# nv-tlabs/ASE

Hardware: AMD Instinct MI355X
Metric: ASE PPO-update samples/sec (4096 envs x horizon 32) (higher is better)
Workload: dtype f16; 1 GPU; BASELINE configs[1]: ASE agent, 4096 envs x horizon 32, obs 253 / act 31 / amp obs 1400 / latent 64, [1024,1024,512] MLPs + disc + shared-trunk encoder, minibatch 16384 (amp 4096) x 6 mini-epochs = 48 optimisation steps per update; random-init weights; precision_choice=auto without an oracle leg: the first candidate, replay=program, parallelism=single GPU

## Files before the change

ase_amd/csrc/gemm_nt_kernels.h:

```cpp
#pragma once
#include "gemm_nt.h"
#include <stdlib.h>
#include <utility>

namespace {

using namespace ase_nt;

typedef uint32_t u32x4 __attribute__((ext_vector_type(4)));
template <int N, typename F, int... I> __device__ __forceinline__ void static_for_impl(F&& f, std::integer_sequence<int, I...>) {
    (f(std::integral_constant<int, I>{}), ...);
}
template <int N, typename F> __device__ __forceinline__ void static_for(F&& f) { static_for_impl<N>(f, std::make_integer_sequence<int, N>{}); }

template <typename T> struct Mma;

template <typename T> struct Mma16 {
    typedef typename V16<T>::x8 x8;
    template <int FM, int FN, int RB, bool SW = false>
    static __device__ __forceinline__ void tile(const char* sA, const char* sB, int lane, f32x16 (&acc)[FM][FN]) {
        const int r = lane & 31, h = lane >> 5, sw = lds_swz<RB>(r);
#pragma unroll
        for (int ks = 0; ks < RB / 32; ++ks) {
            x8 a[FM], b[FN];
            const int off = r * RB + (((ks * 2 + h) ^ sw) << 4);
#pragma unroll
            for (int i = 0; i < FM; ++i)
                a[i] = *reinterpret_cast<const x8*>(sA + i * 32 * RB + off);
#pragma unroll
            for (int j = 0; j < FN; ++j)
                b[j] = *reinterpret_cast<const x8*>(sB + j * 32 * RB + off);
#pragma unroll
            for (int i = 0; i < FM; ++i)
#pragma unroll
                for (int j = 0; j < FN; ++j) {
                    if constexpr (SW) acc[i][j] = mfma16<T>(b[j], a[i], acc[i][j]);
                    else acc[i][j] = mfma16<T>(a[i], b[j], acc[i][j]);
                }
        }
    }
};
template <> struct Mma<bf16_t> : Mma16<bf16_t> {};
template <> struct Mma<f16_t> : Mma16<f16_t> {};

template <> struct Mma<float> {
    template <int FM, int FN, int RB>
    static __device__ __forceinline__ void tile(const char* sA, const char* sB, int lane, f32x16 (&acc)[FM][FN]) {
        const int r = lane & 31, h = lane >> 5, sw = lds_swz<RB>(r);
#pragma unroll
        for (int kb = 0; kb < RB / 32; ++kb) {
            f32x4 a[FM], b[FN];
            const int off = r * RB + (((kb * 2 + h) ^ sw) << 4);
#pragma unroll
            for (int i = 0; i < FM; ++i)
                a[i] = *reinterpret_cast<const f32x4*>(sA + i * 32 * RB + off);
#pragma unroll
            for (int j = 0; j < FN; ++j)
                b[j] = *reinterpret_cast<const f32x4*>(sB + j * 32 * RB + off);
#pragma unroll
            for (int e = 0; e < 4; ++e)
#pragma unroll
                for (int i = 0; i < FM; ++i)
#pragma unroll
                    for (int j = 0; j < FN; ++j)
                        acc[i][j] = __builtin_amdgcn_mfma_f32_32x32x2f32(a[i][e], b[j][e], acc[i][j], 0, 0, 0);
        }
    }
};

__device__ __forceinline__ void split_bf16(const f32x4& x0, const f32x4& x1, bf16x8& hi, bf16x8& lo) {
#pragma unroll
    for (int q = 0; q < 4; ++q) {
        hi[q] = (bf16_t)x0[q];
        hi[q + 4] = (bf16_t)x1[q];
        lo[q] = (bf16_t)(x0[q] - (float)hi[q]);
        lo[q + 4] = (bf16_t)(x1[q] - (float)hi[q + 4]);
    }
}

template <> struct Mma<f32s_t> {
    template <int FM, int FN, int RB>
    static __device__ __forceinline__ void tile(const char* sA, const char* sB, int lane, f32x16 (&acc)[FM][FN]) {
        const int r = lane & 31, h = lane >> 5, sw = lds_swz<RB>(r);
#pragma unroll
        for (int ks = 0; ks < RB / 64; ++ks) {
            bf16x8 ah[FM], al[FM], bh[FN], bl[FN];
            const int c0 = ks * 4 + h * 2;
            const int o0 = r * RB + ((c0 ^ sw) << 4), o1 = r * RB + (((c0 + 1) ^ sw) << 4);
#pragma unroll
            for (int i = 0; i < FM; ++i)
                split_bf16(*reinterpret_cast<const f32x4*>(sA + i * 32 * RB + o0),
                           *reinterpret_cast<const f32x4*>(sA + i * 32 * RB + o1), ah[i], al[i]);
#pragma unroll
            for (int j = 0; j < FN; ++j)
                split_bf16(*reinterpret_cast<const f32x4*>(sB + j * 32 * RB + o0),
                           *reinterpret_cast<const f32x4*>(sB + j * 32 * RB + o1), bh[j], bl[j]);
#pragma unroll
            for (int i = 0; i < FM; ++i)
#pragma unroll
                for (int j = 0; j < FN; ++j) {
                    acc[i][j] = __builtin_amdgcn_mfma_f32_32x32x16_bf16(al[i], bh[j], acc[i][j], 0, 0, 0);
                    acc[i][j] = __builtin_amdgcn_mfma_f32_32x32x16_bf16(ah[i], bl[j], acc[i][j], 0, 0, 0);
                    acc[i][j] = __builtin_amdgcn_mfma_f32_32x32x16_bf16(ah[i], bh[j], acc[i][j], 0, 0, 0);
                }
        }
    }
};

__device__ __forceinline__ void split_f16_pair(float x0, float x1, float sa, uint32_t& hi, uint32_t& lo) {
    asm("v_fma_mixlo_f16 %0, %4, %2, 0\n\t"
        "v_fma_mixhi_f16 %0, %4, %3, 0\n\t"
        "v_fma_mixlo_f16 %1, %4, %2, -%0 op_sel_hi:[0,0,1]\n\t"
        "v_fma_mixhi_f16 %1, %4, %3, -%0 op_sel:[0,0,1] op_sel_hi:[0,0,1]"
        : "=&v"(hi), "=&v"(lo)
        : "v"(x0), "v"(x1), "s"(sa));
}
__device__ __forceinline__ void split_f16_fence(u32x4& hi, u32x4& lo) { asm("s_nop 1" : "+v"(hi), "+v"(lo)); }

template <> struct Mma<f32h_t> {
    template <int RB>
    static __device__ __forceinline__ void frag_offsets(int lane, uint32_t a0, uint32_t b0, uint32_t (&fa)[RB / 64][2], uint32_t (&fb)[RB / 64][2]) {
        const int r = lane & 31, h = lane >> 5, sw = lds_swz<RB>(r);
#pragma unroll
        for (int ks = 0; ks < RB / 64; ++ks)
#pragma unroll
            for (int c = 0; c < 2; ++c) {
                const uint32_t o = r * RB + (((ks * 4 + h * 2 + c) ^ sw) << 4);
                fa[ks][c] = a0 + o;
                fb[ks][c] = b0 + o;
                asm volatile("" : "+v"(fa[ks][c]), "+v"(fb[ks][c]));
            }
    }
    template <int FM, int FN, int RB>
    static __device__ __forceinline__ void tile(const char* smem, uint32_t sbuf, const uint32_t (&fa)[RB / 64][2], const uint32_t (&fb)[RB / 64][2],
                                                f32x16 (&acc)[FM][FN], float sa) {
        constexpr int KS = RB / 64, NM = FM * FN * 3, NP = FM * 4;
        constexpr bool PF = FM * FN <= 4;
        f32x4 ax[2][FM][2];
        u32x4 ah[2][FM], al[2][FM];
        f16x8 bh[2][FN], bl[2][FN];
        auto read_a = [&](int ks) {
#pragma unroll
            for (int i = 0; i < FM; ++i)
#pragma unroll
                for (int c = 0; c < 2; ++c) ax[ks & 1][i][c] = *reinterpret_cast<const f32x4*>(smem + (fa[ks][c] + sbuf) + i * 32 * RB);
        };
        auto read_b = [&](int ks) {
#pragma unroll
            for (int j = 0; j < FN; ++j) {
                bh[PF ? ks & 1 : 0][j] = *reinterpret_cast<const f16x8*>(smem + (fb[ks][0] + sbuf) + j * 32 * RB);
                bl[PF ? ks & 1 : 0][j] = *reinterpret_cast<const f16x8*>(smem + (fb[ks][1] + sbuf) + j * 32 * RB);
            }
        };
        auto split_pair = [&](int ks, int q) {
            const int i = q >> 2, c = (q >> 1) & 1, e = (q & 1) * 2;
            uint32_t hi, lo;
            split_f16_pair(ax[ks & 1][i][c][e], ax[ks & 1][i][c][e + 1], sa, hi, lo);
            ah[ks & 1][i][c * 2 + (q & 1)] = hi;
            al[ks & 1][i][c * 2 + (q & 1)] = lo;
        };
        auto fence = [&](int ks) {
#pragma unroll
            for (int i = 0; i < FM; ++i) split_f16_fence(ah[ks & 1][i], al[ks & 1][i]);
        };
        read_a(0);
        read_b(0);
        __builtin_amdgcn_sched_barrier(0);
#pragma unroll
        for (int q = 0; q < NP; ++q) split_pair(0, q);
        fence(0);
#pragma unroll
        for (int ks = 0; ks < KS; ++ks) {
            const bool more = ks + 1 < KS;
            if (more) {
                read_a(ks + 1);
                if constexpr (PF) read_b(ks + 1);
            }
            __builtin_amdgcn_sched_barrier(0);
#pragma unroll
            for (int i = 0; i < FM; ++i)
#pragma unroll
                for (int j = 0; j < FN; ++j)
#pragma unroll
                    for (int t = 0; t < 3; ++t) {
                        const f16x8 a = __builtin_bit_cast(f16x8, t == 0 ? al[ks & 1][i] : ah[ks & 1][i]);
                        const f16x8 b = (t == 1) ? bl[PF ? ks & 1 : 0][j] : bh[PF ? ks & 1 : 0][j];
                        acc[i][j] = __builtin_amdgcn_mfma_f32_32x32x16_f16(a, b, acc[i][j], 0, 0, 0);
                        if (more) {
                            const int m = (i * FN + j) * 3 + t;
                            __builtin_amdgcn_sched_barrier(0);
#pragma unroll
                            for (int q = 0; q < NP; ++q)
                                if (q * NM >= m * NP && q * NM < (m + 1) * NP) split_pair(ks + 1, q);
                            __builtin_amdgcn_sched_barrier(0);
                        }
                    }
            if (more) {
                fence(ks + 1);
                if constexpr (!PF) read_b(ks + 1);
            }
        }
    }
};

template <int PASSES, int RPP, int RB>
__device__ __forceinline__ void nt_stage(const char* const (&src)[PASSES], int64_t koff, char* lds_wave_base) {
#pragma unroll
    for (int i = 0; i < PASSES; ++i)
        __builtin_amdgcn_global_load_lds((gptr_t*)(src[i] + koff), (lptr_t*)(lds_wave_base + i * RPP * RB), 16, 0, 0);
}
template <typename T, int AUXK> struct AuxReg;
template <typename T> struct AuxReg<T, 0> { char v; };
template <> struct AuxReg<bf16_t, 1> { bf16x4 v; };
template <> struct AuxReg<f16_t, 1> { f16x4 v; };
template <> struct AuxReg<float, 1> { f32x4 v; };
template <> struct AuxReg<f32s_t, 1> { f32x4 v; };
template <> struct AuxReg<f32h_t, 1> { f32x4 v; };
template <typename T> struct AuxReg<T, 2> { uint32_t v; };

__device__ __forceinline__ uint32_t or8_dpp(uint32_t x) {
    x |= (uint32_t)__builtin_amdgcn_update_dpp(0, (int)x, 0xB1, 0xF, 0xF, true);
    x |= (uint32_t)__builtin_amdgcn_update_dpp(0, (int)x, 0x4E, 0xF, 0xF, true);
    x |= (uint32_t)__builtin_amdgcn_update_dpp(0, (int)x, 0x141, 0xF, 0xF, true);
    return x;
}

template <typename T, int FM, int FN, int FMC, int FNC, int AUXK>
__device__ __forceinline__ void nt_aux_load(const NTParams& p, int ch, int lane, int mrow0, int ncol0,
                                            AuxReg<T, AUXK> (&dst)[(FMC * 32) / (64 / (FNC * 8))]) {
    constexpr int ELPR = FNC * 8, RPI = 64 / ELPR, NIT = (FMC * 32) / RPI;
    if constexpr (AUXK != 0) {
        const int c4 = lane % ELPR, rsub = lane / ELPR;
        const int jc = (ch / (FM / FMC)) * FNC, ic = (ch % (FM / FMC)) * FMC;
        const int n0 = ncol0 + jc * 32 + c4 * 4;
#pragma unroll
        for (int it = 0; it < NIT; ++it) {
            const int m = mrow0 + ic * 32 + it * RPI + rsub;
            if (n0 < p.N && m < p.M) {
                const int ma = (m >= p.aux_split) ? m - p.aux_delta : m;
                if constexpr (AUXK == 2)
                    dst[it].v = *reinterpret_cast<const uint32_t*>(p.aux + (int64_t)ma * p.ldaux + (n0 >> 5) * 4);
                else
                    dst[it].v = *reinterpret_cast<const decltype(dst[it].v)*>(p.aux + (int64_t)ma * p.ldaux + (int64_t)n0 * sizeof(T));
            }
        }
    }
}

template <typename T, int FM, int FN, int FMC, int FNC, int AUXK, bool PRE = false, bool FUSE = false>
__device__ __forceinline__ double nt_epilogue_impl(const NTParams& p, f32x16 (&acc)[FM][FN], float* slab, int lane,
                                                   int mrow0, int ncol0,
                                                   AuxReg<T, AUXK> (*pre)[(FMC * 32) / (64 / (FNC * 8))] = nullptr) {
    constexpr int WCOLS = FNC * 32, WROWS = FMC * 32;
    const int col_in = lane & 31, row_hi = (lane >> 5) * 4;
    constexpr int ELPR = WCOLS / 4;
    constexpr int RPI = 64 / ELPR;
    constexpr int NIT = WROWS / RPI;
    constexpr int NCH = (FN / FNC) * (FM / FMC);
    constexpr bool AHEAD = AUXK != 0 && sizeof(AuxReg<T, AUXK>) <= 8;
    const int c4 = lane % ELPR, rsub = lane / ELPR;
    AuxReg<T, AUXK> areg[AHEAD ? 2 : 1][NIT];
    bool bad = false;
    double sq = 0.0;

    auto load_aux = [&](int ch, AuxReg<T, AUXK> (&dst)[NIT]) {
        nt_aux_load<T, FM, FN, FMC, FNC, AUXK>(p, ch, lane, mrow0, ncol0, dst);
    };

    if constexpr (PRE) {
#pragma unroll
        for (int it = 0; it < NIT; ++it) areg[0][it] = (*pre)[it];
    } else if constexpr (AUXK != 0) {
        load_aux(0, areg[0]);
    }
#pragma unroll
    for (int ch = 0; ch < NCH; ++ch) {
        const int jc = (ch / (FM / FMC)) * FNC, ic = (ch % (FM / FMC)) * FMC;
        const int n0 = ncol0 + jc * 32 + c4 * 4;
        if constexpr (AHEAD) {
            if (ch + 1 < NCH) load_aux(ch + 1, areg[(ch + 1) & 1]);
        } else if constexpr (AUXK != 0) {
            if (ch > 0) load_aux(ch, areg[0]);
        }
        AuxReg<T, AUXK> (&cur)[NIT] = areg[AHEAD ? (ch & 1) : 0];
#pragma unroll
        for (int jj = 0; jj < FNC; ++jj) {
            const int j = jc + jj;
            const int n = ncol0 + j * 32 + col_in;
            const float bias = (p.bias && n < p.N) ? p.bias[n] : 0.f;
#pragma unroll
            for (int ii = 0; ii < FMC; ++ii) {
#pragma unroll
                for (int e = 0; e < 16; ++e) {
                    float v = p.alpha * acc[ic + ii][j][e] + bias;
                    if (p.act == ASE_ACT_RELU) v = v <= 0.f ? 0.f : v;
                    else if (p.act == ASE_ACT_TANH) v = tanhf(v);
                    slab[(ii * 32 + row_hi + (e & 3) + 8 * (e >> 2)) * WCOLS + jj * 32 + col_in] = v;
                }
            }
        }
        float cs[4] = {0.f, 0.f, 0.f, 0.f};
        f32x4 seed = {0.f, 0.f, 0.f, 0.f};
        if constexpr (FUSE) {
            if (p.seed_w && n0 < p.N) {
#pragma unroll
                for (int q = 0; q < 4; ++q) seed[q] = p.seed_scale * (n0 + q < p.seed_n ? p.seed_w[n0 + q] : 0.f);
            }
        }
        if (n0 < p.N) {
#pragma unroll
            for (int it = 0; it < NIT; ++it) {
                const int row = it * RPI + rsub;
                const int m = mrow0 + ic * 32 + row;
                if (m >= p.M) continue;
                f32x4 v = *reinterpret_cast<const f32x4*>(slab + row * WCOLS + c4 * 4);
                if (p.act >= ASE_ACT_SILU) {
                    if (p.pre_out) {
                        if constexpr (sizeof(T) == 2) {
                            typename V16<T>::x4 zt;
#pragma unroll
                            for (int q = 0; q < 4; ++q) {
                                zt[q] = from_f32<T>(v[q]);
                                bad |= ovf_hit1(zt[q]);
                            }
                            *reinterpret_cast<typename V16<T>::x4*>(p.pre_out + (int64_t)m * p.ldpre + (int64_t)n0 * 2) = zt;
                        } else {
#pragma unroll
                            for (int q = 0; q < 4; ++q) bad |= ovf_hit1(v[q]);
                            *reinterpret_cast<f32x4*>(p.pre_out + (int64_t)m * p.ldpre + (int64_t)n0 * 4) = v;
                        }
                    }
#pragma unroll
                    for (int q = 0; q < 4; ++q) v[q] = act_apply(p.act, v[q]);
                }
                if constexpr (AUXK == 2) {
                    const uint32_t nib = cur[it].v >> (n0 & 31);
#pragma unroll
                    for (int q = 0; q < 4; ++q) v[q] = ((nib >> q) & 1u) ? v[q] : 0.f;
                } else if constexpr (AUXK == 1) {
#pragma unroll
                    for (int q = 0; q < 4; ++q) {
                        const float a = (float)cur[it].v[q];
                        if (p.aux_mode == ASE_AUX_RELU_MASK) v[q] = a > 0.f ? v[q] : 0.f;
                        else if (p.aux_mode == ASE_AUX_TANH_GRAD) v[q] = v[q] * (1.f - a * a);
                        else v[q] = v[q] * act_grad(p.aux_mode >> 8, a);
                    }
                }
                if constexpr (FUSE) {
                    f32x4 sv = v;
                    if (p.seed_w) {
#pragma unroll
                        for (int q = 0; q < 4; ++q) sv[q] = seed[q] * (v[q] > 0.f ? 1.f : 0.f);
                    }
#pragma unroll
                    for (int q = 0; q < 4; ++q) bad |= ovf_hit1(sv[q]);
                    if (p.C) *reinterpret_cast<f32x4*>(p.C + (int64_t)m * p.ldc + (int64_t)n0 * 4) = sv;
                    if (p.twin) {
                        char* t = p.twin + (int64_t)m * p.ldtwin + (int64_t)n0 * 2;
                        if (p.twin_dtype == ASE_F16) {
                            f16x4 o;
#pragma unroll
                            for (int q = 0; q < 4; ++q) o[q] = from_f32<f16_t>(sv[q]);
                            *reinterpret_cast<f16x4*>(t) = o;
                        } else {
                            bf16x4 o;
#pragma unroll
                            for (int q = 0; q < 4; ++q) o[q] = from_f32<bf16_t>(sv[q]);
                            *reinterpret_cast<bf16x4*>(t) = o;
                        }
                    }
                    if (p.sq_acc) {
                        float s = 0.f;
#pragma unroll
                        for (int q = 0; q < 4; ++q) s = __fadd_rn(s, __fmul_rn(sv[q], sv[q]));
                        sq += (double)s;
                    }
                } else if (p.out_f32 || sizeof(T) == 4) {
#pragma unroll
                    for (int q = 0; q < 4; ++q) bad |= ovf_hit1(v[q]);
                    *reinterpret_cast<f32x4*>(p.C + (int64_t)m * p.ldc + (int64_t)n0 * 4) = v;
                } else {
                    typedef typename std::conditional<sizeof(T) == 2, T, bf16_t>::type S;
                    typename V16<S>::x4 o;
#pragma unroll
                    for (int q = 0; q < 4; ++q) {
                        o[q] = from_f32<S>(v[q]);
                        bad |= ovf_hit1(o[q]);
                        v[q] = (float)o[q];
                    }
                    *reinterpret_cast<typename V16<S>::x4*>(p.C + (int64_t)m * p.ldc + (int64_t)n0 * 2) = o;
                }
#pragma unroll
                for (int q = 0; q < 4; ++q) cs[q] += v[q];
                if (p.mask_out) {
                    uint32_t bits = 0;
#pragma unroll
                    for (int q = 0; q < 4; ++q) bits |= (v[q] > 0.f ? 1u : 0u) << q;
                    bits = or8_dpp(bits << (n0 & 31));
                    if ((c4 & 7) == 0) p.mask_out[(int64_t)m * p.ldmask + (n0 >> 5)] = bits;
                }
            }
        }
        if (p.colsum) {
#pragma unroll
            for (int q = 0; q < 4; ++q) {
#pragma unroll
                for (int o = ELPR; o < 64; o <<= 1) cs[q] += __shfl_xor(cs[q], o, 64);
            }
            if (lane < ELPR) {
#pragma unroll
                for (int q = 0; q < 4; ++q)
                    if (n0 + q < p.colsum_n) atomic_add_f32(p.colsum + n0 + q, cs[q]);
            }
        }
    }
    ovf_report(p.alpha_dev, bad);
    return sq;
}

template <typename T, int FM, int FN, int FMC, int FNC, bool FUSE = false>
__device__ __forceinline__ double nt_epilogue(const NTParams& p, f32x16 (&acc)[FM][FN], float* slab, int lane, int mrow0,
                                              int ncol0) {
    if (p.aux_mode == ASE_AUX_NONE) return nt_epilogue_impl<T, FM, FN, FMC, FNC, 0, false, FUSE>(p, acc, slab, lane, mrow0, ncol0);
    if (p.aux_mode == ASE_AUX_RELU_BITS) return nt_epilogue_impl<T, FM, FN, FMC, FNC, 2, false, FUSE>(p, acc, slab, lane, mrow0, ncol0);
    if constexpr (FUSE) return 0.0;
    else return nt_epilogue_impl<T, FM, FN, FMC, FNC, 1>(p, acc, slab, lane, mrow0, ncol0);
}

template <typename T, int FM, int FN, int AUXK, bool MASK>
__device__ __forceinline__ void nt_epilogue_rows_impl(const NTParams& p, f32x16 (&acc)[FM][FN], int lane, int mrow0, int ncol0,
                                                      const uint32_t (&bits)[FM][FN]) {
    const int r = lane & 31, h = lane >> 5;
    const f32x2 al = {p.alpha, p.alpha};
    const float relu_lo = (p.act == ASE_ACT_RELU) ? 0.f : -__builtin_inff();
    uint32_t ovf = 0;
#pragma unroll
    for (int j = 0; j < FN; ++j) {
        f32x4 bias[4];
#pragma unroll
        for (int g = 0; g < 4; ++g) {
            if (p.bias) bias[g] = *reinterpret_cast<const f32x4*>(p.bias + ncol0 + j * 32 + 8 * g + 4 * h);
            else bias[g] = f32x4{0.f, 0.f, 0.f, 0.f};
        }
#pragma unroll
        for (int i = 0; i < FM; ++i) {
            const int m = mrow0 + i * 32 + r;
            const bool row_ok = m < p.M;
            char* crow = p.C + (int64_t)m * p.ldc + (int64_t)(ncol0 + j * 32) * 2 + h * 16;
            uint32_t pk[4][2];
            const uint32_t mb = rows_frag<T, AUXK, MASK>(acc[i][j], bias, AUXK == 2 ? bits[i][j] >> (4 * h) : 0u, al, relu_lo, h, pk);
#pragma unroll
            for (int g = 0; g < 4; g += 2) {
                const auto s0 = __builtin_amdgcn_permlane32_swap(pk[g][0], pk[g + 1][0], false, false);
                const auto s1 = __builtin_amdgcn_permlane32_swap(pk[g][1], pk[g + 1][1], false, false);
                if (row_ok) *reinterpret_cast<uint4*>(crow + 8 * g * 2) = make_uint4(s0[0], s1[0], s0[1], s1[1]);
                ovf = ovf_fold(ovf_fold(ovf_fold(ovf_fold(ovf, s0[0]), s1[0]), s0[1]), s1[1]);
            }
            if constexpr (MASK) {
                const auto w = __builtin_amdgcn_permlane32_swap(mb, mb, false, false);
                if (row_ok && h == 0) p.mask_out[(int64_t)m * p.ldmask + ((ncol0 + j * 32) >> 5)] = w[0] | w[1];
            }
        }
    }
    ovf_report(p.alpha_dev, ovf_hit<T>(ovf));
}

template <typename T, int FM, int FN, int AUXK>
__device__ __forceinline__ void nt_epilogue_rows(const NTParams& p, f32x16 (&acc)[FM][FN], int lane, int mrow0, int ncol0,
                                                 const uint32_t (&bits)[FM][FN]) {
    if (ncol0 >= p.N) return;
    if (p.mask_out) nt_epilogue_rows_impl<T, FM, FN, AUXK, true>(p, acc, lane, mrow0, ncol0, bits);
    else nt_epilogue_rows_impl<T, FM, FN, AUXK, false>(p, acc, lane, mrow0, ncol0, bits);
}

template <int WGM, int WGN, int FM, int FN, int RB, int S, int A_PASSES, int B_PASSES>
__device__ __forceinline__ void nt_h3_loop(const NTParams& p, char* smem, const char* const (&srcA)[A_PASSES], const char* const (&srcB)[B_PASSES],
                                           int lane, int wid, int wm, int wn, int nk, f32x16 (&acc)[FM][FN]) {
    constexpr int BM = WGM * FM * 32, BN = WGN * FN * 32, RPW = 64 / (RB / 16), RPP = WGM * WGN * RPW, P = A_PASSES + B_PASSES;
    constexpr int kBuf = (BM + BN) * RB;
    uint32_t fa[RB / 64][2], fb[RB / 64][2];
    Mma<f32h_t>::template frag_offsets<RB>(lane, (wm * FM * 32) * RB, (BM + wn * FN * 32) * RB, fa, fb);
    const bool fits32 = (int64_t)p.M * p.lda < (int64_t)0x7FFFFFFF && (int64_t)p.N * p.ldb < (int64_t)0x7FFFFFFF;
    const i32x4 rsA = raw_buffer(p.A), rsB = raw_buffer(p.B);
    const uint32_t lds0 = __builtin_amdgcn_readfirstlane((uint32_t)(uintptr_t)smem + wid * RPW * RB);
    uint32_t voffA[A_PASSES], voffB[B_PASSES];
#pragma unroll
    for (int i = 0; i < A_PASSES; ++i) voffA[i] = (uint32_t)(srcA[i] - p.A);
#pragma unroll
    for (int i = 0; i < B_PASSES; ++i) voffB[i] = (uint32_t)(srcB[i] - p.B);
    auto stage = [&](int t, int b) {
        const uint32_t dst = lds0 + (uint32_t)b * kBuf;
        if (fits32) {
            const uint32_t soff = (uint32_t)t * RB;
            static_for<A_PASSES>([&](auto i) { lds_dma16<i.value * RPP * RB, true>(dst, voffA[i.value], rsA, soff); });
            static_for<B_PASSES>([&](auto i) { lds_dma16<(BM + i.value * RPP) * RB, true>(dst, voffB[i.value], rsB, soff); });
        } else {
            const int64_t koff = (int64_t)t * RB;
            static_for<A_PASSES>([&](auto i) { lds_dma16_global<i.value * RPP * RB>(dst, srcA[i.value] + koff); });
            static_for<B_PASSES>([&](auto i) { lds_dma16_global<(BM + i.value * RPP) * RB>(dst, srcB[i.value] + koff); });
        }
    };
#pragma unroll
    for (int t = 0; t < S - 1; ++t)
        if (t < nk) stage(t, t);
    __builtin_amdgcn_s_waitcnt(0xC07F);
    int buf = 0, prev = S - 1;
    for (int kt = 0; kt < nk; ++kt) {
        if (kt + S - 2 < nk) wait_vmcnt<P*(S - 2)>();
        else wait_vmcnt<0>();
        __builtin_amdgcn_s_barrier();
        if (kt + S - 1 < nk) stage(kt + S - 1, prev);
        Mma<f32h_t>::template tile<FM, FN, RB>(smem, (uint32_t)buf * kBuf, fa, fb, acc, p.sa);
        prev = buf;
        buf = (buf + 1 == S) ? 0 : buf + 1;
    }
}

template <typename T, int WGM, int WGN, int FM, int FN, int RB, int S, int WPE = 1, bool SW = false, bool FUSE = false>
__global__ __launch_bounds__(WGM * WGN * 64, WPE) void gemm_nt_kernel(NTParams p) {
    constexpr int BM = WGM * FM * 32, BN = WGN * FN * 32;
    constexpr int BK = RB / (int)sizeof(T);
    constexpr int LPR = RB / 16;
    constexpr int RPW = 64 / LPR;
    constexpr int RPP = WGM * WGN * RPW;
    constexpr int A_PASSES = BM / RPP, B_PASSES = BN / RPP;
    constexpr int P = A_PASSES + B_PASSES;
    static_assert(BM % RPP == 0 && BN % RPP == 0, "tile rows must be a multiple of the rows staged per pass");
    extern __shared__ __attribute__((aligned(16))) char smem[];
    constexpr int kBuf = (BM + BN) * RB;
    if (p.alpha_dev) p.alpha *= *p.alpha_dev;

    const int tid = threadIdx.x, lane = tid & 63, wid = tid >> 6;
    const int wm = wid / WGN, wn = wid % WGN;
    const int nwg = p.tiles_m * p.tiles_n;
    const int tile = xcd_remap(blockIdx.x, nwg);
    const int bm0 = (tile / p.tiles_n) * BM, bn0 = (tile % p.tiles_n) * BN;

    const int srow = tid / LPR, sslot = tid % LPR;
    const char* srcA[A_PASSES];
    const char* srcB[B_PASSES];
#pragma unroll
    for (int i = 0; i < A_PASSES; ++i) {
        const int r = i * RPP + srow;
        srcA[i] = p.A + (int64_t)min(bm0 + r, p.M - 1) * p.lda + ((sslot ^ lds_swz<RB>(r)) << 4);
    }
#pragma unroll
    for (int i = 0; i < B_PASSES; ++i) {
        const int r = i * RPP + srow;
        srcB[i] = p.B + (int64_t)min(bn0 + r, p.N - 1) * p.ldb + ((sslot ^ lds_swz<RB>(r)) << 4);
    }
    char* const ldsA = smem + (wid * RPW) * RB;
    char* const ldsB = ldsA + BM * RB;

    f32x16 acc[FM][FN];
#pragma unroll
    for (int i = 0; i < FM; ++i)
#pragma unroll
        for (int j = 0; j < FN; ++j)
#pragma unroll
            for (int e = 0; e < 16; ++e) acc[i][j][e] = 0.f;

    uint32_t row_bits[FM][FN];
    auto load_bits = [&]() {
        if (p.aux_mode == ASE_AUX_RELU_BITS && bn0 + wn * FN * 32 < p.N) {
#pragma unroll
            for (int i = 0; i < FM; ++i) {
                const int m = min(bm0 + wm * FM * 32 + i * 32 + (lane & 31), p.M - 1);
                const int ma = (m >= p.aux_split) ? m - p.aux_delta : m;
                const uint32_t* w = reinterpret_cast<const uint32_t*>(p.aux + (int64_t)ma * p.ldaux) + ((bn0 + wn * FN * 32) >> 5);
#pragma unroll
                for (int j = 0; j < FN; ++j) row_bits[i][j] = w[j];
            }
        }
    };
    if constexpr (SW && S == 2) load_bits();

    const int nk = p.K / BK;
    if constexpr (std::is_same<T, f32h_t>::value) {
        nt_h3_loop<WGM, WGN, FM, FN, RB, S>(p, smem, srcA, srcB, lane, wid, wm, wn, nk, acc);
    } else {
#pragma unroll
        for (int t = 0; t < S - 1; ++t) {
            if (t < nk) {
                nt_stage<A_PASSES, RPP, RB>(srcA, (int64_t)t * RB, ldsA + t * kBuf);
                nt_stage<B_PASSES, RPP, RB>(srcB, (int64_t)t * RB, ldsB + t * kBuf);
            }
        }
        int buf = 0;
        for (int kt = 0; kt < nk; ++kt) {
            if (kt + S - 2 < nk) wait_vmcnt<P*(S - 2)>();
            else wait_vmcnt<0>();
            __builtin_amdgcn_s_barrier();
            if (kt + S - 1 < nk) {
                const int nb = (buf == 0) ? S - 1 : buf - 1;
                nt_stage<A_PASSES, RPP, RB>(srcA, (int64_t)(kt + S - 1) * RB, ldsA + nb * kBuf);
                nt_stage<B_PASSES, RPP, RB>(srcB, (int64_t)(kt + S - 1) * RB, ldsB + nb * kBuf);
            }
            const char* sA = smem + buf * kBuf + (wm * FM * 32) * RB;
            const char* sB = smem + buf * kBuf + (BM + wn * FN * 32) * RB;
            if constexpr (SW && sizeof(T) == 2) Mma<T>::template tile<FM, FN, RB, true>(sA, sB, lane, acc);
            else Mma<T>::template tile<FM, FN, RB>(sA, sB, lane, acc);
            buf = (buf + 1 == S) ? 0 : buf + 1;
        }
    }
    if constexpr (SW) {
        if constexpr (S != 2) load_bits();
        if constexpr (sizeof(T) == 2) {
            if (p.aux_mode == ASE_AUX_RELU_BITS) nt_epilogue_rows<T, FM, FN, 2>(p, acc, lane, bm0 + wm * FM * 32, bn0 + wn * FN * 32, row_bits);
            else nt_epilogue_rows<T, FM, FN, 0>(p, acc, lane, bm0 + wm * FM * 32, bn0 + wn * FN * 32, row_bits);
        }
        return;
    }
    __syncthreads();

    constexpr int FNC = (FN > 2) ? 2 : FN;
    float* slab = reinterpret_cast<float*>(smem) + wid * (FM * 32 * FNC * 32);
    const double sq = nt_epilogue<T, FM, FN, FM, FNC, FUSE>(p, acc, slab, lane, bm0 + wm * FM * 32, bn0 + wn * FN * 32);
    if constexpr (FUSE) {
        if (p.sq_acc) {
            const double w = wave_sum(sq);
            __syncthreads();
            double* red = reinterpret_cast<double*>(smem);
            if (lane == 0) red[wid] = w;
            __syncthreads();
            if (tid == 0) {
                double t = 0.0;
                for (int i = 0; i < WGM * WGN; ++i) t += red[i];
                double scale = p.sq_scale;
                if (p.sq_dyn) scale *= (double)*p.sq_dyn;
                atomic_add_f64(p.sq_acc, t * scale);
            }
        }
    }
}

template <typename T, int WGM, int WGN, int FM, int FN, int RB, int S, int WPE = 1, bool SW = false, bool FUSE = false>
int launch_nt(const NTParams& p0, hipStream_t stream) {
    constexpr int BM = WGM * FM * 32, BN = WGN * FN * 32;
    constexpr int ring = S * (BM + BN) * RB;
    constexpr int slab = WGM * WGN * (FM * 32) * ((FN > 2 ? 2 : FN) * 32) * 4;
    constexpr int lds = ring > slab ? ring : slab;
    static_assert(lds <= 160 * 1024, "LDS budget");
    constexpr auto kern = gemm_nt_kernel<T, WGM, WGN, FM, FN, RB, S, WPE, SW, FUSE>;
    if (const int rc = ase_dynamic_lds<kern>("gemm_nt", lds)) return rc;
    NTParams p = p0;
    p.tiles_m = (p.M + BM - 1) / BM;
    p.tiles_n = (p.N + BN - 1) / BN;
    ASE_LAUNCH(kern, dim3(p.tiles_m * p.tiles_n), dim3(WGM * WGN * 64), lds, stream, p);
    ASE_CHECK_LAUNCH("gemm_nt");
    return ASE_OK;
}


struct NT8Lane {
    uint32_t voff[4][2];
    uint32_t dst[4][2];
    int roff[4];
    i32x4 rsA, rsB;
};

template <int KIND>
__device__ __forceinline__ void nt8_piece(const NT8Lane& L, int g, int tile) {
    constexpr bool isB = (KIND == 1 || KIND == 2);
    lds_dma16(__builtin_amdgcn_readfirstlane(L.dst[KIND][g] + (uint32_t)(tile & 1) * 65536u), L.voff[KIND][g], isB ? L.rsB : L.rsA,
              (uint32_t)tile * 128u);
}

template <int KIND>
__device__ __forceinline__ void nt8_issue(const NT8Lane& L, int tile) {
#pragma unroll
    for (int g = 0; g < 2; ++g) nt8_piece<KIND>(L, g, tile);
}

__device__ __forceinline__ void nt8_read(i32x4 (&f)[4], const char* base, const NT8Lane& L) {
#pragma unroll
    for (int ks = 0; ks < 4; ++ks) f[ks] = *reinterpret_cast<const i32x4*>(base + L.roff[ks]);
}

template <typename T, int KIND, bool SW, int NA = 2>
__device__ __forceinline__ void nt8_mma_issue(f32x16& c0, f32x16& c1, const i32x4 (&a0)[4], const i32x4 (&a1)[4],
                                              const i32x4 (&b)[4], const NT8Lane& L, int tile, bool live) {
#pragma unroll
    for (int ks = 0; ks < 4; ++ks) {
        if (ks == 3) NT8_BARRIER();
        c0 = nt8_mfma<T, SW>(a0[ks], b[ks], c0);
        if constexpr (NA == 2) c1 = nt8_mfma<T, SW>(a1[ks], b[ks], c1);
        if (ks == 0 || ks == 2) {
            __builtin_amdgcn_sched_barrier(0);
            if (live) nt8_piece<KIND>(L, ks >> 1, tile);
            __builtin_amdgcn_sched_barrier(0);
        }
    }
    __builtin_amdgcn_sched_barrier(0);
    __builtin_amdgcn_s_setprio(0);
    __builtin_amdgcn_sched_barrier(0);
}

template <typename T, bool TAIL, bool SW, int NI = 4>
__device__ __forceinline__ void nt8_ktile(int t, int nk, const NT8Lane& L, const char* aP, const char* bP,
                                          f32x16 (&acc)[NI][2], i32x4 (&a0)[4], i32x4 (&a1)[4], i32x4 (&b0)[4],
                                          i32x4 (&b1)[4]) {
    constexpr int RB = 128;
    const int U = 4 * nk;
    const bool l1 = !TAIL || t + 1 < nk, l2 = !TAIL || t + 2 < nk;
    nt8_read(b0, bP, L);
    nt8_read(a0, aP, L);
    nt8_read(a1, aP + 32 * RB, L);
    if (!TAIL) wait_dma_units<3>();
    else wait_dma_units_rt(min(U, 4 * t + 6) - (4 * t + 3));
    nt8_sync_in();
    nt8_mma_issue<T, 2, SW>(acc[0][0], acc[1][0], a0, a1, b0, L, t + 1, l1);
    nt8_read(b1, bP + 32 * RB, L);
    if (!TAIL) wait_dma_units<3>();
    else wait_dma_units_rt(min(U, 4 * t + 7) - (4 * t + 4));
    nt8_sync_in();
    nt8_mma_issue<T, 3, SW>(acc[0][1], acc[1][1], a0, a1, b1, L, t + 1, l1);
    nt8_read(a0, aP + 64 * RB, L);
    if constexpr (NI == 4) nt8_read(a1, aP + 96 * RB, L);
    nt8_sync_in();
    nt8_mma_issue<T, 0, SW, NI - 2>(acc[2][1], acc[NI - 1][1], a0, a1, b1, L, t + 2, l2);
    if (!TAIL) wait_dma_units<3>();
    else if (t + 1 < nk) wait_dma_units_rt(min(U, 4 * t + 9) - (4 * t + 6));
    nt8_sync_in();
    nt8_mma_issue<T, 1, SW, NI - 2>(acc[2][0], acc[NI - 1][0], a0, a1, b0, L, t + 2, l2);
}


template <typename T, bool SW, int BM = 256>
__global__ __launch_bounds__(512) void gemm_nt8_kernel(NTParams p) {
    static_assert(sizeof(T) == 2, "the phased kernel takes the 16-bit storage types");
    static_assert(BM == 256 || (BM == 192 && SW), "192-row tiles come with the row-per-lane epilogue");
    constexpr int RB = 128, BN = 256, BK = 64, WM = BM / 2, NI = WM / 32;
    constexpr int kBuf = 512 * RB;
    extern __shared__ __attribute__((aligned(16))) char smem[];
    if (p.alpha_dev) p.alpha *= *p.alpha_dev;

    const int tid = threadIdx.x, lane = tid & 63;
    const int wid = __builtin_amdgcn_readfirstlane(tid >> 6);
    const int wr = wid >> 2, wc = wid & 3;
    const int nwg = p.tiles_m * p.tiles_n;
    const int tile = xcd_remap(blockIdx.x, nwg);
    const int bm0 = (tile / p.tiles_n) * BM, bn0 = (tile % p.tiles_n) * BN;

    NT_PROF_STAMP(p.prof, tid, blockIdx.x * 4 + 0, false);
    NT8Lane L;
    {
        const int lr = lane >> 3, slot = lane & 7;
#pragma unroll
        for (int g = 0; g < 2; ++g) {
            const int ra = g * WM + wid * 8;
            const int rb = (g * 2 + (wid >> 2)) * 64 + (wid & 3) * 8;
            const int ra1 = BM == 256 ? ra + 64 : (wid >> 2) * WM + 64 + (wid & 3) * 8;
            const int rows[4] = {ra, rb, rb + 32, ra1};
#pragma unroll
            for (int kind = 0; kind < 4; ++kind) {
                const int r = rows[kind] + lr;
                const bool isB = (kind == 1 || kind == 2);
                const int64_t grow = isB ? min(bn0 + r, p.N - 1) : min(bm0 + r, p.M - 1);
                L.voff[kind][g] = (uint32_t)(grow * (isB ? p.ldb : p.lda)) + (uint32_t)((slot ^ lds_swz<RB>(r)) << 4);
                L.dst[kind][g] = (uint32_t)(uintptr_t)smem + (isB ? BM * RB : 0) + rows[kind] * RB;
            }
        }
        const int r = lane & 31, h = lane >> 5, sw = lds_swz<RB>(r);
#pragma unroll
        for (int ks = 0; ks < 4; ++ks) L.roff[ks] = r * RB + (((ks * 2 + h) ^ sw) << 4);
        L.rsA = raw_buffer(p.A);
        L.rsB = raw_buffer(p.B);
    }

    f32x16 acc[NI][2];
#pragma unroll
    for (int i = 0; i < NI; ++i)
#pragma unroll
        for (int j = 0; j < 2; ++j)
#pragma unroll
            for (int e = 0; e < 16; ++e) acc[i][j][e] = 0.f;

    AuxReg<T, 2> pre_bits[16];
    uint32_t row_bits[NI][2];
    if constexpr (!SW) {
        if (p.aux_mode == ASE_AUX_RELU_BITS) nt_aux_load<T, 4, 2, 2, 2, 2>(p, 0, lane, bm0 + wr * WM, bn0 + wc * 64, pre_bits);
    }

    const int nk = p.K / BK;
    nt8_issue<0>(L, 0);
    nt8_issue<1>(L, 0);
    nt8_issue<2>(L, 0);
    nt8_issue<3>(L, 0);
    if (nk > 1) {
        nt8_issue<0>(L, 1);
        nt8_issue<1>(L, 1);
    }
    bool mask_dma = false;
    if constexpr (SW) {
        mask_dma = p.aux_mode == ASE_AUX_RELU_BITS && bn0 + wc * 64 < p.N;
        if (mask_dma) {
            char* mlds = smem + 2 * kBuf + wid * 1024;
#pragma unroll
            for (int i = 0; i < NI; ++i) {
                const int m = bm0 + wr * WM + i * 32 + (lane & 31);
                const int ma = (m >= p.aux_split) ? m - p.aux_delta : m;
                const uint32_t* w = reinterpret_cast<const uint32_t*>(p.aux + (int64_t)min(ma, p.M - 1) * p.ldaux) +
                                    ((bn0 + wc * 64) >> 5) + (lane >> 5);
                __builtin_amdgcn_global_load_lds((gptr_t*)w, (lptr_t*)(mlds + i * 256), 4, 0, 0);
            }
        }
    }
    if (nk > 1) {
        if (mask_dma) wait_vmcnt<8 + NI>(); else wait_dma_units<4>();
    } else {
        if (mask_dma) wait_vmcnt<4 + NI>(); else wait_dma_units<2>();
    }
    NT8_BARRIER();
    NT_PROF_STAMP(p.prof, tid, blockIdx.x * 4 + 1, p.prof_clk);
    if (wr == 1) NT8_BARRIER();

    i32x4 a0[4], a1[4], b0[4], b1[4];
    const int aoff = wr * WM * RB, boff = BM * RB + wc * 64 * RB;
    int t = 0;
    for (; t + 2 < nk; ++t) {
        const char* buf = smem + (t & 1) * kBuf;
        nt8_ktile<T, false, SW, NI>(t, nk, L, buf + aoff, buf + boff, acc, a0, a1, b0, b1);
    }
    for (; t < nk; ++t) {
        const char* buf = smem + (t & 1) * kBuf;
        nt8_ktile<T, true, SW, NI>(t, nk, L, buf + aoff, buf + boff, acc, a0, a1, b0, b1);
    }
    if (wr == 0) NT8_BARRIER();
    __syncthreads();
    NT_PROF_STAMP(p.prof, tid, blockIdx.x * 4 + 2, p.prof_clk);

    float* slab = reinterpret_cast<float*>(smem) + wid * (64 * 64);
    if constexpr (SW) {
        if (p.aux_mode == ASE_AUX_RELU_BITS) {
            const uint32_t* mw = reinterpret_cast<const uint32_t*>(smem + 2 * kBuf + wid * 1024);
#pragma unroll
            for (int i = 0; i < NI; ++i) {
                row_bits[i][0] = mw[i * 64 + (lane & 31)];
                row_bits[i][1] = mw[i * 64 + 32 + (lane & 31)];
            }
            nt8_epilogue_rows<T, 2, 2, NI>(p, acc, lane, bm0 + wr * WM, bn0 + wc * 64, row_bits);
        } else nt8_epilogue_rows<T, 0, 2, NI>(p, acc, lane, bm0 + wr * WM, bn0 + wc * 64, row_bits);
    } else if constexpr (BM == 256) {
        if (p.aux_mode == ASE_AUX_RELU_BITS)
            nt_epilogue_impl<T, 4, 2, 2, 2, 2, true>(p, acc, slab, lane, bm0 + wr * 128, bn0 + wc * 64, &pre_bits);
        else
            nt_epilogue<T, 4, 2, 2, 2>(p, acc, slab, lane, bm0 + wr * 128, bn0 + wc * 64);
    }
    NT_PROF_CLOSE(p.prof, tid, blockIdx.x * 4 + 3);
}

template <typename T, bool SW = false, int BM = 256> int launch_nt8(const NTParams& p0, hipStream_t stream) {
    constexpr int lds = 2 * 512 * 128 + (SW ? 8 * 1024 : 0);
    constexpr auto kern = gemm_nt8_kernel<T, SW, BM>;
    if (const int rc = ase_dynamic_lds<kern>("gemm_nt8", lds)) return rc;
    NTParams p = p0;
    p.prof = g_nt_prof;
    p.prof_clk = g_nt_prof_clk;
    p.tiles_m = (p.M + BM - 1) / BM;
    p.tiles_n = (p.N + 255) / 256;
    ASE_LAUNCH(kern, dim3(p.tiles_m * p.tiles_n), dim3(512), lds, stream, p);
    ASE_CHECK_LAUNCH("gemm_nt8");
    return ASE_OK;
}

}
#include "gemm_nt4.h"
namespace {

inline bool rows_epi(const NTParams& p, int wave_cols) {
    return !p.out_f32 && p.N % wave_cols == 0 && p.colsum == nullptr && p.act <= ASE_ACT_RELU &&
           (p.mask_out == nullptr || p.act == ASE_ACT_RELU) &&
           (p.aux_mode == ASE_AUX_NONE || p.aux_mode == ASE_AUX_RELU_BITS);
}

template <typename T> int dispatch_nt(const NTParams& p, hipStream_t s) {
    const bool k128 = (p.K * (int)sizeof(T)) % 128 == 0;
    const bool fits32 = (int64_t)p.M * p.lda < (int64_t)0x7FFFFFFF && (int64_t)p.N * p.ldb < (int64_t)0x7FFFFFFF;
    int choice = nt_choice(p.M, p.N, p.K, (int)sizeof(T), sizeof(T) == 2);
    if ((choice == 2 || choice == 6) && !fits32) choice = 3;
    if constexpr (std::is_same<T, f32h_t>::value) {
        if (p.seed_w || p.twin || p.sq_acc) {
            switch (choice) {
                case 0: return launch_nt<T, 2, 2, 1, 1, 64, 4, 1, false, true>(p, s);
                case 2: case 3: case 6:
                    if (k128) return launch_nt<T, 4, 2, 2, 4, 128, 2, 1, false, true>(p, s);
                    return launch_nt<T, 4, 2, 2, 4, 64, 4, 1, false, true>(p, s);
                case 4: return launch_nt<T, 2, 2, 1, 2, 128, 2, 2, false, true>(p, s);
                case 5: return launch_nt<T, 2, 2, 1, 1, 128, 4, 2, false, true>(p, s);
                default:
                    if (k128) return launch_nt<T, 2, 2, 2, 2, 128, 2, 2, false, true>(p, s);
                    return launch_nt<T, 2, 2, 2, 2, 64, 4, 2, false, true>(p, s);
            }
        }
    }
    switch (choice) {
        case 0: return launch_nt<T, 2, 2, 1, 1, 64, 4>(p, s);
        case 6:
            if constexpr (sizeof(T) == 2) if (rows_epi(p, 64)) return launch_nt8<T, true, 192>(p, s);
            [[fallthrough]];
        case 2:
            if constexpr (sizeof(T) == 2) {
                if (p.M >= 65536 && rows_epi(p, 128)) return launch_nt4<T>(p, s);
                if (rows_epi(p, 64)) return launch_nt8<T, true>(p, s);
                return launch_nt8<T, false>(p, s);
            }
            [[fallthrough]];
        case 3:
            if (k128) return launch_nt<T, 4, 2, 2, 4, 128, 2>(p, s);
            return launch_nt<T, 4, 2, 2, 4, 64, 4>(p, s);
        case 4:
            if constexpr (sizeof(T) == 2) if (rows_epi(p, 64)) return launch_nt<T, 2, 2, 1, 2, 128, 2, 2, true>(p, s);
            return launch_nt<T, 2, 2, 1, 2, 128, 2, 2>(p, s);
        case 5:
            if constexpr (sizeof(T) == 2) if (rows_epi(p, 32)) return launch_nt<T, 2, 2, 1, 1, 128, 4, 2, true>(p, s);
            return launch_nt<T, 2, 2, 1, 1, 128, 4, 2>(p, s);
        default:
            if constexpr (sizeof(T) == 2) if (k128 && rows_epi(p, 64)) return launch_nt<T, 2, 2, 2, 2, 128, 2, 1, true>(p, s);
            if (k128) return launch_nt<T, 2, 2, 2, 2, 128, 2>(p, s);
            return launch_nt<T, 2, 2, 2, 2, 64, 4>(p, s);
    }
}

}
```

Measured before the change: 1.853 million samples/s.

## Route 16-bit NT GEMM through buffer-DMA ring loop with prefetched LDS fragments

Generalizes the f32h ring loop (32-bit buffer-resource LDS DMA staging with precomputed offsets) into a tile-agnostic nt_ring_loop and uses it for f16/bf16 NT GEMMs except the smallest tile shape. Adds a 16-bit Mma tile variant that precomputes per-lane swizzled fragment offsets once and double-buffers LDS fragment reads across k-substeps, with sched barriers so the next reads overlap the current MFMAs. This aims to cut per-iteration address arithmetic and LDS-read latency stalls in the main GEMM loop, at the cost of extra VGPRs for double-buffered fragments, which may hurt occupancy.

```diff
diff --git a/ase_amd/csrc/gemm_nt_kernels.h b/ase_amd/csrc/gemm_nt_kernels.h
--- a/ase_amd/csrc/gemm_nt_kernels.h
+++ b/ase_amd/csrc/gemm_nt_kernels.h
@@ -37,6 +37,51 @@
                     if constexpr (SW) acc[i][j] = mfma16<T>(b[j], a[i], acc[i][j]);
                     else acc[i][j] = mfma16<T>(a[i], b[j], acc[i][j]);
                 }
+        }
+    }
+    template <int RB>
+    static __device__ __forceinline__ void frag_offsets(int lane, uint32_t (&fo)[RB / 32]) {
+        const int r = lane & 31, h = lane >> 5, sw = lds_swz<RB>(r);
+#pragma unroll
+        for (int ks = 0; ks < RB / 32; ++ks) {
+            fo[ks] = r * RB + (((ks * 2 + h) ^ sw) << 4);
+            asm volatile("" : "+v"(fo[ks]));
+        }
+    }
+    template <int FM, int FN, int RB, bool SW = false>
+    static __device__ __forceinline__ void tile(const char* smem, uint32_t sa, uint32_t sb, const uint32_t (&fo)[RB / 32], f32x16 (&acc)[FM][FN]) {
+        constexpr int KS = RB / 32;
+        constexpr bool PF = FM * FN < 4;
+        x8 a[2][FM], b[2][FN];
+        auto read_a = [&](int ks) {
+#pragma unroll
+            for (int i = 0; i < FM; ++i) a[ks & 1][i] = *reinterpret_cast<const x8*>(smem + (fo[ks] + sa) + i * 32 * RB);
+        };
+        auto read_b = [&](int ks) {
+#pragma unroll
+            for (int j = 0; j < FN; ++j) b[PF ? ks & 1 : 0][j] = *reinterpret_cast<const x8*>(smem + (fo[ks] + sb) + j * 32 * RB);
+        };
+        read_a(0);
+        read_b(0);
+#pragma unroll
+        for (int ks = 0; ks < KS; ++ks) {
+            const bool more = ks + 1 < KS;
+            if (more) {
+                read_a(ks + 1);
+                if constexpr (PF) read_b(ks + 1);
+            }
+            __builtin_amdgcn_sched_barrier(0);
+#pragma unroll
+            for (int i = 0; i < FM; ++i)
+#pragma unroll
+                for (int j = 0; j < FN; ++j) {
+                    if constexpr (SW) acc[i][j] = mfma16<T>(b[PF ? ks & 1 : 0][j], a[ks & 1][i], acc[i][j]);
+                    else acc[i][j] = mfma16<T>(a[ks & 1][i], b[PF ? ks & 1 : 0][j], acc[i][j]);
+                }
+            __builtin_amdgcn_sched_barrier(0);
+            if constexpr (!PF) {
+                if (more) read_b(ks + 1);
+            }
         }
     }
 };
@@ -473,13 +518,11 @@
     else nt_epilogue_rows_impl<T, FM, FN, AUXK, false>(p, acc, lane, mrow0, ncol0, bits);
 }
 
-template <int WGM, int WGN, int FM, int FN, int RB, int S, int A_PASSES, int B_PASSES>
-__device__ __forceinline__ void nt_h3_loop(const NTParams& p, char* smem, const char* const (&srcA)[A_PASSES], const char* const (&srcB)[B_PASSES],
-                                           int lane, int wid, int wm, int wn, int nk, f32x16 (&acc)[FM][FN]) {
+template <int WGM, int WGN, int FM, int FN, int RB, int S, int A_PASSES, int B_PASSES, typename Tile>
+__device__ __forceinline__ void nt_ring_loop(const NTParams& p, char* smem, const char* const (&srcA)[A_PASSES], const char* const (&srcB)[B_PASSES],
+                                             int wid, int nk, Tile&& tile) {
     constexpr int BM = WGM * FM * 32, BN = WGN * FN * 32, RPW = 64 / (RB / 16), RPP = WGM * WGN * RPW, P = A_PASSES + B_PASSES;
     constexpr int kBuf = (BM + BN) * RB;
-    uint32_t fa[RB / 64][2], fb[RB / 64][2];
-    Mma<f32h_t>::template frag_offsets<RB>(lane, (wm * FM * 32) * RB, (BM + wn * FN * 32) * RB, fa, fb);
     const bool fits32 = (int64_t)p.M * p.lda < (int64_t)0x7FFFFFFF && (int64_t)p.N * p.ldb < (int64_t)0x7FFFFFFF;
     const i32x4 rsA = raw_buffer(p.A), rsB = raw_buffer(p.B);
     const uint32_t lds0 = __builtin_amdgcn_readfirstlane((uint32_t)(uintptr_t)smem + wid * RPW * RB);
@@ -510,11 +553,13 @@
         else wait_vmcnt<0>();
         __builtin_amdgcn_s_barrier();
         if (kt + S - 1 < nk) stage(kt + S - 1, prev);
-        Mma<f32h_t>::template tile<FM, FN, RB>(smem, (uint32_t)buf * kBuf, fa, fb, acc, p.sa);
+        tile((uint32_t)buf * kBuf);
         prev = buf;
         buf = (buf + 1 == S) ? 0 : buf + 1;
     }
 }
+
+template <typename T, int FM, int FN, int RB> constexpr bool nt_ring16() { return sizeof(T) == 2 && !(RB == 64 && FM * FN == 1); }
 
 template <typename T, int WGM, int WGN, int FM, int FN, int RB, int S, int WPE = 1, bool SW = false, bool FUSE = false>
 __global__ __launch_bounds__(WGM * WGN * 64, WPE) void gemm_nt_kernel(NTParams p) {
@@ -577,7 +622,18 @@
 
     const int nk = p.K / BK;
     if constexpr (std::is_same<T, f32h_t>::value) {
-        nt_h3_loop<WGM, WGN, FM, FN, RB, S>(p, smem, srcA, srcB, lane, wid, wm, wn, nk, acc);
+        uint32_t fa[RB / 64][2], fb[RB / 64][2];
+        Mma<f32h_t>::template frag_offsets<RB>(lane, (wm * FM * 32) * RB, (BM + wn * FN * 32) * RB, fa, fb);
+        nt_ring_loop<WGM, WGN, FM, FN, RB, S>(p, smem, srcA, srcB, wid, nk, [&](uint32_t sbuf) {
+            Mma<f32h_t>::template tile<FM, FN, RB>(smem, sbuf, fa, fb, acc, p.sa);
+        });
+    } else if constexpr (nt_ring16<T, FM, FN, RB>()) {
+        uint32_t fo[RB / 32];
+        Mma<T>::template frag_offsets<RB>(lane, fo);
+        const uint32_t a0 = __builtin_amdgcn_readfirstlane((wm * FM * 32) * RB), b0 = __builtin_amdgcn_readfirstlane((BM + wn * FN * 32) * RB);
+        nt_ring_loop<WGM, WGN, FM, FN, RB, S>(p, smem, srcA, srcB, wid, nk, [&](uint32_t sbuf) {
+            Mma<T>::template tile<FM, FN, RB, SW>(smem, a0 + sbuf, b0 + sbuf, fo, acc);
+        });
     } else {
 #pragma unroll
         for (int t = 0; t < S - 1; ++t) {
```

New measurement: 1.857 million samples/s (median of 4 runs). No clear change (+0.2%).
